# SamuelGong/FLASHE

Measured on AMD Instinct MI355X. Metric: ciphertexts/sec (enc+agg+dec), 1e7-elem vector; achieved HBM GB/s fraction, higher is better.
Workload: dtype u128

## Files before the change

flashe_amd/csrc/abi.hip:

```cpp
#include "ctx.h"
#include "blockpool.h"

#include <algorithm>
#include <cstdarg>
#include <cstdio>
#include <cstdlib>
#include <cmath>
#include <cstring>
#include <mutex>
#include <new>
#include <string>
#include <vector>

using namespace flashe;

namespace {

struct AesTables {
    uint8_t sbox[256];
    uint32_t te0[256];
    AesTables()
    {
        uint8_t alog[256], lg[256];
        uint8_t x = 1;
// ... 330 lines not shown
    ctx->env.rkw_dev = ctx->rkw_dev;
    if ((e = hipMalloc(&ctx->rkp_dev, 15 * 64 * 4)) != hipSuccess) return bail(FLASHE_ENOMEM, "hipMalloc(rkp)", e);
    ctx->env.rkp_dev = ctx->rkp_dev;
    if ((e = hipHostMalloc(reinterpret_cast<void **>(&ctx->err_flag_host), 64, hipHostMallocMapped)) != hipSuccess)
        return bail(FLASHE_ENOMEM, "hipHostMalloc(error flag)", e);
    *ctx->err_flag_host = 0;
    if ((e = hipHostGetDevicePointer(reinterpret_cast<void **>(&ctx->env.err_flag), ctx->err_flag_host, 0)) != hipSuccess)
        return bail(FLASHE_EIO, "hipHostGetDevicePointer", e);
    expand_key(key, &ctx->env.rk);
    if (upload_key_words(ctx) != FLASHE_OK) {
        g_create_error = ctx->err;
        (void)flashe_ctx_destroy(ctx);
        return FLASHE_EIO;
    }
    ctx->env.prf_backend = PRF_AUTO;
    ctx->env.hybrid_bs_permille = 300;
    if ((e = hipStreamCreateWithFlags(&ctx->env.stream2, hipStreamNonBlocking)) != hipSuccess) return bail(FLASHE_EIO, "hipStreamCreate(2)", e);
    if ((e = hipEventCreateWithFlags(&ctx->env.ev_fork, hipEventDisableTiming)) != hipSuccess) return bail(FLASHE_EIO, "hipEventCreate", e);
    if ((e = hipEventCreateWithFlags(&ctx->env.ev_join, hipEventDisableTiming)) != hipSuccess) return bail(FLASHE_EIO, "hipEventCreate", e);
    if (const char *be = getenv("FLASHE_PRF_BACKEND")) {
        if (!strcmp(be, "table")) ctx->env.prf_backend = PRF_TABLE;
#ifdef FLASHE_WITH_BITSLICE
        else if (!strcmp(be, "bitslice")) ctx->env.prf_backend = PRF_BITSLICE;
        else if (!strcmp(be, "hybrid")) ctx->env.prf_backend = PRF_HYBRID;
        else if (!strcmp(be, "bitslice16")) ctx->env.prf_backend = PRF_BITSLICE16;
#endif
    }
#ifdef FLASHE_TUNING
    if (const char *pm = getenv("FLASHE_HYBRID_BS_PERMILLE")) ctx->env.hybrid_bs_permille = atoi(pm);
#endif
    ctx->env.use_chain = 1;
    if (const char *ch = getenv("FLASHE_CHAIN")) ctx->env.use_chain = atoi(ch) != 0;
    if (const char *dm = getenv("FLASHE_CHAIN_DMASK")) ctx->chain_dmask_on = atoi(dm) != 0;
    *out = ctx;
    return FLASHE_OK;
}

int flashe_ctx_destroy(flashe_ctx *ctx)
{
    if (!ctx) return FLASHE_EINVAL;
    (void)hipSetDevice(ctx->device);
    if (ctx->env.stream) (void)hipStreamSynchronize(ctx->env.stream);
    for (flashe_ctx::Buf *b : {&ctx->summaries, &ctx->stream_tmp, &ctx->acc_tmp[0], &ctx->acc_tmp[1], &ctx->sp_ws, &ctx->bounds, &ctx->mt_ws, &ctx->codec_tab, &ctx->prep_enc.add,
                               &ctx->prep_enc.minus, &ctx->prep_dec.add, &ctx->prep_dec.minus, &ctx->chain_dmask.d})
        if (b->p) (void)hipFree(b->p);
    if (ctx->staging) { ctx->staging->destroy(); delete ctx->staging; ctx->staging = nullptr; }
    if (ctx->te0_dev) (void)hipFree(ctx->te0_dev);
    if (ctx->rkw_dev) { (void)hipMemset(ctx->rkw_dev, 0, 256); (void)hipFree(ctx->rkw_dev); }
    if (ctx->rkp_dev) { (void)hipMemset(ctx->rkp_dev, 0, 15 * 64 * 4); (void)hipFree(ctx->rkp_dev); }
    wipe(&ctx->env.rk, sizeof(ctx->env.rk));
    if (ctx->err_flag_host) (void)hipHostFree(ctx->err_flag_host);
    if (ctx->env.stream2) { (void)hipStreamSynchronize(ctx->env.stream2); (void)hipStreamDestroy(ctx->env.stream2); }
    if (ctx->env.ev_fork) (void)hipEventDestroy(ctx->env.ev_fork);
    if (ctx->env.ev_join) (void)hipEventDestroy(ctx->env.ev_join);
    for (hipEvent_t &ev : ctx->ev_copy) if (ev) (void)hipEventDestroy(ev);
    if (ctx->own_stream && ctx->env.stream) (void)hipStreamDestroy(ctx->env.stream);
    delete ctx;
    return FLASHE_OK;
}

int flashe_ctx_set_key(flashe_ctx *ctx, const uint8_t key[32])
{
    if (!ctx || !key) return FLASHE_EINVAL;
    HIP_TRY(ctx, hipSetDevice(ctx->device));
    HIP_TRY(ctx, hipStreamSynchronize(ctx->env.stream));
    wipe(&ctx->env.rk, sizeof(ctx->env.rk));
// ... 1848 lines not shown
{
    CHECK_CTX(ctx);
    if (n_layers < 0 || (n_layers && (!n || !k))) return fail(ctx, FLASHE_EINVAL, "sparsify_batch: bad arguments");
    if (n_layers == 0) return FLASHE_OK;
    if (ctx->capturing) return fail(ctx, FLASHE_EINVAL, "sparsify_batch: not inside a graph capture (the layer table is uploaded synchronously)");
    uint64_t total = 0, total_k = 0;
    for (int l = 0; l < n_layers; l++) {
        if (n[l] >= (1ull << 32)) return fail(ctx, FLASHE_EINVAL, "sparsify_batch: layer %d: n must be < 2^32", l);
        if (k[l] > n[l]) return fail(ctx, FLASHE_EINVAL, "sparsify_batch: layer %d: k (%llu) > n (%llu)", l, static_cast<unsigned long long>(k[l]),
                                     static_cast<unsigned long long>(n[l]));
        total += n[l]; total_k += k[l];
    }
    if (total == 0 || total_k == 0) return FLASHE_OK;
    if (!x_dev || !loc_dev || !vals_dev) return fail(ctx, FLASHE_EINVAL, "null vector");
    std::vector<unsigned char> desc(sparsify_batch_desc_bytes(n_layers));
    const uint64_t blocks = sparsify_batch_layout(n_layers, n, k, desc.data());
    if (blocks >= (1ull << 32)) return fail(ctx, FLASHE_EINVAL, "sparsify_batch: too many elements");
    int rc = ensure(ctx, ctx->sp_ws, sparsify_batch_workspace_bytes(n_layers, blocks));
    if (rc) return rc;
    HIP_TRY(ctx, hipMemcpyAsync(ctx->sp_ws.p, desc.data(), desc.size(), hipMemcpyHostToDevice, ctx->env.stream));
    HIP_TRY(ctx, hipStreamSynchronize(ctx->env.stream));
    HIP_TRY(ctx, launch_sparsify_batch(ctx->env, n_layers, blocks, x_dev, x_is_f64 != 0, residual_dev, loc_dev, vals_dev, ctx->sp_ws.p));
    return FLASHE_OK;
}

#ifdef FLASHE_TUNING
int flashe_tune_span_prf_cycles(flashe_ctx *ctx, unsigned long long *out8, int reset)
{
    CHECK_CTX(ctx);
    HIP_TRY(ctx, hipStreamSynchronize(ctx->env.stream));
    HIP_TRY(ctx, flashe::span_prf_cycles(out8, reset != 0));
    return FLASHE_OK;
}
int flashe_tune_reduce_decrypt_probe(flashe_ctx *ctx, int variant, uint32_t iter, uint32_t add_idx, uint32_t minus_idx, int C,
                                     const uint64_t *const *cts_dev, uint64_t n, uint64_t *out_dev)
{
    CHECK_CTX(ctx);
    if (!cts_dev || !out_dev) return fail(ctx, FLASHE_EINVAL, "null vector");
    HIP_TRY(ctx, launch_reduce_decrypt_probe(ctx->env, variant, iter, add_idx, minus_idx, C, cts_dev, n, out_dev));
    return FLASHE_OK;
}
#endif

}
```

flashe_amd/csrc/kernels.h:

```cpp
#pragma once
#include <hip/hip_runtime.h>
#include <stdint.h>

namespace flashe {

struct RoundKeys { uint32_t w[60]; };

struct CodecLayer {
    uint64_t start;
    const void *x;
    double p0, p1, p2;
    int x_is_f64, pad_;
};
struct Codec {
    const void *x;
    const double *u;
    double alpha, scale, den;
    int x_is_f64, n_layers;
    double *fout;
    double ac, two_a, uden;
    const CodecLayer *layers;
    uint64_t k0;
};

struct LaunchEnv {
    hipStream_t stream;
    int num_cus;
    const uint32_t *te0_dev;
    const uint32_t *rkw_dev;
    const uint32_t *rkp_dev;
    RoundKeys rk;
    int b;
    int prf_backend;
    hipStream_t stream2;
    hipEvent_t ev_fork, ev_join;
    int hybrid_bs_permille;
    const Codec *codec;
    uint32_t *err_flag;
    int use_chain;
    int elem32 = 0;
};

enum { PRF_AUTO = 0, PRF_TABLE = 1, PRF_BITSLICE = 2, PRF_HYBRID = 3, PRF_BITSLICE16 = 4 };

constexpr int kMaxIdx = 96;
hipError_t launch_prf(const LaunchEnv &env, uint32_t iter,
                      const uint32_t *add, int n_add, const uint32_t *minus, int n_minus,
                      uint64_t n, uint32_t n_jobs, uint64_t first, uint64_t count,
                      const uint64_t *in_dev, int in_limbs, uint64_t *out_dev);

constexpr int kMaxBatch = 32;
constexpr int kMaxUniformBatch = 128;
hipError_t launch_prf_batch(const LaunchEnv &env, uint32_t iter, bool dbl, int n_vec, const uint32_t *idx,
                            const uint64_t *const *in_dev, int in_limbs, uint64_t *const *out_dev, uint64_t n,
                            uint32_t n_jobs);
hipError_t launch_prf_batch_sum(const LaunchEnv &env, uint32_t iter, int n_vec, const uint32_t *idx, const uint64_t *const *in_dev,
                                int in_limbs, uint64_t *const *out_dev, uint64_t *sum_out_dev, uint64_t n, uint32_t n_jobs, uint64_t first,
                                uint64_t count, uint64_t *dmask_dev = nullptr);
hipError_t launch_prf_batch_range(const LaunchEnv &env, uint32_t iter, bool dbl, int n_vec, const uint32_t *idx, const uint64_t *const *in_dev,
                                  int in_limbs, uint64_t *const *out_dev, uint64_t n, uint32_t n_jobs, uint64_t first, uint64_t count);

struct PrfJob {
    uint32_t add_idx, minus_idx;
    uint64_t first, count;
    const uint64_t *in_dev;
    int in_limbs;
    uint64_t *out_dev;
    uint32_t n_in = 1;
    uint64_t in_stride = 0;
    uint64_t *sum_out_dev = nullptr;
};
hipError_t launch_prf_jobs(const LaunchEnv &env, uint32_t iter, bool dbl, int n_entries, const PrfJob *jobs, uint64_t n,
                           uint32_t n_jobs);
// ... 36 lines not shown
hipError_t launch_aggregate_packed(const LaunchEnv &env, int C, const uint64_t *const *ops,
                                   uint64_t n_limbs, uint64_t total_bits, uint64_t *out_dev,
                                   uint32_t *summaries_dev);

hipError_t launch_packed_probe(const LaunchEnv &env, uint64_t n_limbs, const uint64_t *x_dev, uint64_t *info_dev);
hipError_t launch_packed_add_carry(const LaunchEnv &env, uint64_t n_limbs, uint64_t total_bits, uint64_t cin, uint64_t *x_dev);
hipError_t launch_packed_resolve_carry(const LaunchEnv &env, uint64_t n_limbs, uint64_t total_bits, const uint64_t *infos_dev, int n_below,
                                       uint64_t *x_dev, int stride_words = 3);

hipError_t launch_pack(const LaunchEnv &env, uint64_t n, const uint64_t *in_dev, uint64_t *out_dev);
hipError_t launch_unpack(const LaunchEnv &env, uint64_t n, const uint64_t *in_dev, uint64_t *out_dev);

hipError_t launch_fill(const LaunchEnv &env, uint64_t n, uint64_t lo, uint64_t hi, uint64_t *out_dev);
hipError_t launch_scatter(const LaunchEnv &env, uint64_t total, uint64_t k, const uint32_t *loc_dev,
                          const uint64_t *vals_dev, uint64_t *out_dev, bool accumulate,
                          uint64_t sub_lo = 0, uint64_t sub_hi = 0);
constexpr int kMaxScatter = 64;
#ifndef FLASHE_SPAN_FUSED
#define FLASHE_SPAN_FUSED 1752
#endif
constexpr int kSpanReduce = 4096, kSpanFused = FLASHE_SPAN_FUSED;
uint64_t span_count(uint64_t total, int span);
inline size_t span_table_words(uint64_t total, int C) { return static_cast<size_t>(span_count(total, kSpanFused) + 1) * static_cast<size_t>(C); }
hipError_t launch_span_reduce(const LaunchEnv &env, int C, const uint32_t *const *loc_dev, const uint64_t *const *vals_dev,
                              const uint64_t *k, const uint64_t *sub, uint64_t base_lo, uint64_t base_hi, uint64_t total,
                              uint32_t *start_dev, const uint64_t *src_dev, bool negate, uint64_t *out_dev, bool bounds_ready = false);
hipError_t launch_span_bounds(const LaunchEnv &env, int C, const uint32_t *const *loc_dev, const uint64_t *k, uint64_t total, uint32_t *start_reduce_dev,
                              uint32_t *start_fused_dev);
hipError_t launch_span_prf(const LaunchEnv &env, uint32_t iter, int C, const uint32_t *idx, const uint32_t *const *loc_dev, const uint64_t *k,
                           const uint64_t *const *pt_dev, int pt_limbs, uint64_t *const *ct_dev, const uint64_t *sub, uint64_t base_lo, uint64_t base_hi,
                           uint64_t total, const uint32_t *start_dev, const uint64_t *src_dev, bool negate, uint64_t *out_dev, uint64_t first, uint64_t count);
#ifdef FLASHE_TUNING
hipError_t span_prf_cycles(unsigned long long *out8, bool reset);
#endif
hipError_t launch_sparse_edge_prf(const LaunchEnv &env, uint32_t iter, int nc, uint32_t c0, const uint32_t *const *loc_with_neighbours,
                                  const uint64_t *k_with_neighbours, uint64_t *const *va_dev, uint64_t *const *vm_dev);
hipError_t launch_shared_positions(const LaunchEnv &env, int nc, const uint32_t *const *loc_with_next, const uint64_t *k_with_next,
                                   unsigned long long *count_dev);
hipError_t launch_sel_accumulate(const LaunchEnv &env, uint64_t total, const uint8_t *sel_dev,
                                 const uint64_t *stream_dev, uint64_t *out_dev);

Codec codec_quantize_front(const void *x_dev, bool is_f64, double alpha, int bits, const double *u_dev);
void codec_unquantize_back(Codec *c, double alpha, int bits, int num_clients, double *out_dev);
CodecLayer codec_layer_front(uint64_t start, const void *x_dev, bool is_f64, double alpha, int bits);
CodecLayer codec_layer_back(uint64_t start, double alpha, int bits, int num_clients);
hipError_t launch_shift(const LaunchEnv &env, uint64_t n, void *x_dev, bool is_f64, double shift, bool wide);
int moments_grid(const LaunchEnv &env, uint64_t n);
hipError_t launch_moment(const LaunchEnv &env, uint64_t n, const void *x_dev, bool is_f64, double center, int pow, double *part_dev);
hipError_t launch_quantize(const LaunchEnv &env, uint64_t n, const void *x_dev, bool is_f64, double alpha, int bits,
                           const double *u_dev, uint64_t *q_dev);
hipError_t launch_unquantize_model(const LaunchEnv &env, uint64_t count, const uint64_t *v_dev, const Codec &cq, double *out_dev);
hipError_t launch_unquantize(const LaunchEnv &env, uint64_t n, const uint64_t *v_dev, int v_limbs, double alpha, int bits,
                             int num_clients, double *out_dev);
hipError_t launch_batch(const LaunchEnv &env, uint64_t n, const uint64_t *vals_dev, int field_bits, uint64_t *out_dev);
struct BatchLayer {
    uint64_t elem_start;
    uint64_t value_start;
    uint64_t size;
    const void *x;
    double p0, p1, p2;
    int x_is_f64, pad_;
};
hipError_t launch_quantize_batch_model(const LaunchEnv &env, const BatchLayer *layers_dev, int n_layers, int field_bits, const double *u_dev,
                                       uint64_t n_elems, uint64_t *out_dev);
hipError_t launch_unbatch_unquantize_model(const LaunchEnv &env, const BatchLayer *layers_dev, int n_layers, int field_bits, const uint64_t *in_dev,
                                           uint64_t n_values, double *out_dev);
// ... 25 lines not shown
```

flashe_amd/csrc/kernels.hip:

```cpp
#include "device_common.h"

namespace flashe {

struct IdxLists {
    uint32_t add[kMaxIdx];
    uint32_t minus[kMaxIdx];
};

struct PrfParams {
    const uint64_t *in;
    uint64_t *out;
    const uint32_t *te0;
    uint64_t n;
    uint64_t first, count;
    uint64_t blk_first, blk_count;
    uint64_t mask_lo, mask_hi;
    uint32_t iter;
    int in_limbs;
    int n_add, n_minus;
    uint32_t n_jobs;
    int b, m;
    Codec cq;
};

// ... 206 lines not shown
constexpr int kMaxLinks = 128;
struct ChainTable {
    uint64_t first[kMaxChains], count[kMaxChains];
    uint64_t wend[kMaxChains];
    uint16_t link0[kMaxChains], sbase[kMaxChains];
    uint8_t len[kMaxChains];
    uint8_t flags[kMaxChains];
    uint32_t idx[kMaxLinks + kMaxChains];
    const uint64_t *in[kMaxLinks];
    uint64_t *out[kMaxLinks];
    uint64_t *sum_out[kMaxChains];
};

__device__ __forceinline__ CtrPrefix load_prefix(const uint32_t *pre_lds, int s)
{
    const uint4 v = *reinterpret_cast<const uint4 *>(pre_lds + 4 * s);
    return CtrPrefix{{static_cast<uint32_t>(__builtin_amdgcn_readfirstlane(v.x)), static_cast<uint32_t>(__builtin_amdgcn_readfirstlane(v.y)),
                      static_cast<uint32_t>(__builtin_amdgcn_readfirstlane(v.z)), static_cast<uint32_t>(__builtin_amdgcn_readfirstlane(v.w))}};
}

__device__ __forceinline__ void loads_landed(const u128 &a, const u128 &b)
{
    asm volatile("" ::"v"(static_cast<uint64_t>(a)), "v"(static_cast<uint64_t>(a >> 64)), "v"(static_cast<uint64_t>(b)),
                 "v"(static_cast<uint64_t>(b >> 64)));
}

template <class T> __device__ __forceinline__ void swap_regs(T &a, T &b) { const T t = a; a = b; b = t; }

__device__ __forceinline__ uint64_t uniform64(uint64_t v)
{
    return static_cast<uint32_t>(__builtin_amdgcn_readfirstlane(static_cast<uint32_t>(v))) |
           (static_cast<uint64_t>(static_cast<uint32_t>(__builtin_amdgcn_readfirstlane(static_cast<uint32_t>(v >> 32)))) << 32);
}

template <int THREADS, bool SUM, bool CODEC>
__global__ __launch_bounds__(THREADS) void prf_chain_kernel(const RoundKeys rk, const ChainTable tb, int n_chains, int all_half_arg,
                                                              uint32_t iter0, uint64_t mask_lo, uint64_t mask_hi,
                                                              const uint32_t *__restrict__ te0, const Codec cq)
{
    constexpr bool DMASK = false;
    uint64_t *const dmask = nullptr;
#include "prf_chain_body.inc"
}

template <int THREADS>
__global__ __launch_bounds__(THREADS) void prf_chain_dmask_kernel(const RoundKeys rk, const ChainTable tb, int n_chains, int all_half_arg,
                                                                    uint32_t iter0, uint64_t mask_lo, uint64_t mask_hi,
                                                                    const uint32_t *__restrict__ te0, uint64_t *__restrict__ dmask)
{
    constexpr bool SUM = true, CODEC = false, DMASK = true;
    const Codec cq{};
#include "prf_chain_body.inc"
}

__device__ __forceinline__ uint64_t extract64(u128 S, int sh)
{
    return sh >= 128 ? 0ull : static_cast<uint64_t>(S >> sh);
}

constexpr int kSmallThreads = 1024;
constexpr int kTch = 8;

__global__ __launch_bounds__(kSmallThreads) void prf_small_kernel(const RoundKeys rk, const PrfParams p, const IdxLists lists)
{
    const uint32_t iter = p.iter + p.te0[kIterShiftWord];
    __shared__ uint32_t tab[kTabWords];
// ... 1508 lines not shown
static hipError_t launch_small_chains(const LaunchEnv &env, uint32_t iter, int n_chains, const PrfChain *chains, uint64_t n, uint32_t n_jobs);

#ifndef FLASHE_CHAIN_QUARTER_DEFAULT
#define FLASHE_CHAIN_QUARTER_DEFAULT 1
#endif
hipError_t launch_prf_chains(const LaunchEnv &env, uint32_t iter, int n_chains, const PrfChain *chains, uint64_t n, uint32_t n_jobs)
{
    if (env.b <= 64) return launch_small_chains(env, iter, n_chains, chains, n, n_jobs);
    struct Piece { const PrfChain *ch; int l0, l1; uint64_t tiles; };
    std::vector<Piece> pieces;
    uint64_t total_tiles = 0;
    bool summed = false;
    uint64_t *dmask = nullptr;
    for (int i = 0; i < n_chains; i++) {
        const PrfChain &c = chains[i];
        if (c.dmask_dev && (n_chains != 1 || !c.sum_out_dev || c.single)) return hipErrorInvalidValue;
        dmask = c.dmask_dev;
        if (c.count == 0 || c.n_out == 0) continue;
        if (((c.first + c.count - 1) >> 32) != (c.first >> 32)) return hipErrorNotSupported;
        if (c.sum_out_dev) { if (c.n_out > kMaxLinks) return hipErrorNotSupported; summed = true; }
        const uint64_t tiles = (c.first + c.count - (c.first & ~255ull) + 255) / 256;
        pieces.push_back(Piece{&c, 0, c.n_out, tiles});
        total_tiles += tiles;
    }
    if (pieces.empty()) return hipSuccess;
    const uint64_t waves = static_cast<uint64_t>(env.num_cus) * (kPrfThreads / 64);
    bool all_half = total_tiles < 2 * waves;
    static const bool tune = FLASHE_TUNE_ENV("FLASHE_CHAIN_TUNE") != nullptr;
    int force_parts = 0, force_grid = 0, probe = 0;
    if (tune) {
        if (const char *e = FLASHE_TUNE_ENV("FLASHE_CHAIN_HALF")) all_half = atoi(e) != 0;
        if (const char *e = FLASHE_TUNE_ENV("FLASHE_CHAIN_PARTS")) force_parts = atoi(e);
        if (const char *e = FLASHE_TUNE_ENV("FLASHE_CHAIN_GRID")) force_grid = atoi(e);
        if (const char *e = FLASHE_TUNE_ENV("FLASHE_CHAIN_PROBE")) probe = atoi(e) == 1 ? 0x100 : atoi(e) == 2 ? 0x200 : 0;
    }
    bool only_single = true;
    for (const Piece &pc : pieces) only_single &= pc.ch->single && !pc.ch->sum_out_dev;
    int single_parts = 0;
    if (only_single && all_half && !force_parts && !(tune && FLASHE_TUNE_ENV("FLASHE_CHAIN_HALF"))) {
        single_parts = static_cast<int>(std::min<uint64_t>((2 * waves + total_tiles - 1) / total_tiles, kMaxChains / pieces.size()));
        if (single_parts < 1) single_parts = 1;
        uint64_t cut_tiles = 0;
        for (const Piece &pc : pieces) cut_tiles += pc.tiles * static_cast<uint64_t>(std::min(single_parts, pc.l1));
        all_half = 2 * cut_tiles < waves;
    }
    uint64_t cuttable_tiles = 0, fixed_items = 0;
    for (const Piece &pc : pieces) {
        if (pc.l1 >= 8 && !pc.ch->sum_out_dev) cuttable_tiles += pc.tiles;
        else fixed_items += 2 * pc.tiles;
    }
    bool quarter = !env.codec && !summed && !single_parts && all_half && 4 * total_tiles <= waves && !force_parts && FLASHE_CHAIN_QUARTER_DEFAULT;
    if (tune) {
        if (const char *e = FLASHE_TUNE_ENV("FLASHE_CHAIN_QUARTER")) quarter = atoi(e) != 0 && !env.codec && !summed && !single_parts && all_half;
    }
    std::vector<Piece> cut;
    for (const Piece &pc : pieces) {
        int parts = (pc.l1 + kMaxLinks - 1) / kMaxLinks;
        if (single_parts) {
            parts = std::max(parts, std::min(single_parts, pc.l1));
        } else if (quarter && !pc.ch->sum_out_dev && pc.l1 >= 2) {
            uint64_t cut4 = 0, fixed4 = 0;
            for (const Piece &o : pieces) (o.l1 >= 2 && !o.ch->sum_out_dev ? cut4 : fixed4) += 4 * o.tiles;
            const uint64_t want = fixed4 < waves ? std::max<uint64_t>((waves - fixed4) / cut4, 1) : 1;
            parts = std::max<int>(parts, static_cast<int>(std::min<uint64_t>(want, static_cast<uint64_t>(pc.l1))));
            parts = std::min(parts, std::max(1, kMaxChains / static_cast<int>(pieces.size())));
            parts = std::max(parts, (pc.l1 + kMaxLinks - 1) / kMaxLinks);
        } else if (all_half && 2 * total_tiles < waves && !pc.ch->sum_out_dev) {
// ... 15 lines not shown
    size_t at = 0;
    while (at < cut.size()) {
        ChainTable tb{};
        int nc = 0, links = 0, streams = 0;
        uint64_t wend = 0, tiles = 0;
        while (at < cut.size() && nc < kMaxChains && links + (cut[at].l1 - cut[at].l0) <= kMaxLinks) {
            const Piece &pc = cut[at++];
            const PrfChain &c = *pc.ch;
            const int len = pc.l1 - pc.l0, ns = len + (c.single ? 0 : 1);
            tb.first[nc] = c.first; tb.count[nc] = c.count;
            tb.link0[nc] = static_cast<uint16_t>(links); tb.sbase[nc] = static_cast<uint16_t>(streams);
            tb.len[nc] = static_cast<uint8_t>(len);
            tb.flags[nc] = static_cast<uint8_t>((c.single ? 1 : 0) | (c.in_limbs == 2 ? 2 : 0));
            tb.sum_out[nc] = c.sum_out_dev;
            for (int s = 0; s < ns; s++) tb.idx[streams + s] = c.idx[pc.l0 + s];
            for (int l = 0; l < len; l++) {
                tb.in[links + l] = c.in_dev ? c.in_dev[pc.l0 + l] : nullptr;
                tb.out[links + l] = c.out_dev[pc.l0 + l];
            }
            wend += pc.tiles * static_cast<uint64_t>(ns);
            tb.wend[nc] = wend;
            tiles += pc.tiles;
            links += len; streams += ns; nc++;
        }
        const uint64_t items = quarter ? 4 * tiles : all_half ? 2 * tiles : tiles, cus = static_cast<uint64_t>(env.num_cus);
        int grid = static_cast<int>(items < cus ? items : cus);
        if (force_grid > 0) grid = force_grid;
        Codec cq{};
        if (env.codec) {
            if (cut.size() != 1 || cut[0].l1 - cut[0].l0 != 1) return hipErrorInvalidValue;
            cq = *env.codec;
        }
        if (env.codec && summed) return hipErrorInvalidValue;
        if (dmask)
            hipLaunchKernelGGL((prf_chain_dmask_kernel<kPrfThreads>), dim3(grid), dim3(kPrfThreads), 0, env.stream, env.rk, tb, nc,
                               (all_half ? 1 : 0) | (quarter ? 4 : 0) | probe, iter, lo, hi, env.te0_dev, dmask);
        else if (env.codec)
            hipLaunchKernelGGL((prf_chain_kernel<kPrfThreads, false, true>), dim3(grid), dim3(kPrfThreads), 0, env.stream, env.rk, tb, nc,
                               (all_half ? 1 : 0) | (quarter ? 4 : 0) | probe, iter, lo, hi, env.te0_dev, cq);
        else if (summed)
            hipLaunchKernelGGL((prf_chain_kernel<kPrfThreads, true, false>), dim3(grid), dim3(kPrfThreads), 0, env.stream, env.rk, tb, nc,
                               (all_half ? 1 : 0) | (quarter ? 4 : 0) | probe, iter, lo, hi, env.te0_dev, cq);
        else
            hipLaunchKernelGGL((prf_chain_kernel<kPrfThreads, false, false>), dim3(grid), dim3(kPrfThreads), 0, env.stream, env.rk, tb, nc,
                               (all_half ? 1 : 0) | (quarter ? 4 : 0) | probe, iter, lo, hi, env.te0_dev, cq);
        const hipError_t e = hipGetLastError();
        if (e != hipSuccess) return e;
    }
    return hipSuccess;
}

static SmallParams small_params_of(const LaunchEnv &env, uint32_t iter, uint64_t n, uint32_t n_jobs)
{
    SmallParams p{};
    p.n = n; p.n_jobs = n_jobs; p.iter = iter; p.b = env.b; p.m = 128 / env.b; p.te0 = env.te0_dev;
    { static const int v = FLASHE_TUNE_ENV("FLASHE_SMALL_DIRECT") ? atoi(FLASHE_TUNE_ENV("FLASHE_SMALL_DIRECT")) : 1; p.no_direct = v == 0 ? 1 : v == 2 ? 2 : 0; }
    { static const int v = FLASHE_TUNE_ENV("FLASHE_SMALL_FIXED") ? atoi(FLASHE_TUNE_ENV("FLASHE_SMALL_FIXED")) : 1; p.no_fixed_width = v == 0; }
    p.m_magic = static_cast<uint32_t>(((1ull << 32) + p.m - 1) / p.m);
    uint64_t hi;
    masks_of(env.b, &p.mask_lo, &hi);
    unsigned __int128 top = 0;
    for (int t = 0; t < p.m; t++) top |= static_cast<unsigned __int128>(1) << (env.b * t + env.b - 1);
    p.top_lo = static_cast<uint64_t>(top); p.top_hi = static_cast<uint64_t>(top >> 64);
    const uint64_t mm = p.m, d = n / n_jobs, nb1 = (d + 1 + mm - 1) / mm, nb0 = d ? (d + mm - 1) / mm : 0;
    p.nb1_magic = nb1 > 1 && nb1 < (1ull << 32) ? static_cast<uint32_t>((1ull << 32) / nb1) : 0;
    p.nb0_magic = nb0 > 1 && nb0 < (1ull << 32) ? static_cast<uint32_t>((1ull << 32) / nb0) : 0;
    return p;
}

hipError_t launch_small_reduce_decrypt(const LaunchEnv &env, uint32_t iter, uint32_t add_idx, bool has_minus, uint32_t minus_idx, uint64_t n,
                                       uint32_t n_jobs, uint64_t first, uint64_t count, int C, const uint64_t *const *ops, uint64_t *agg_out_dev,
                                       uint64_t *out_dev, int out_elem_bytes)
{
    if (env.b > 64 || env.codec || n >= (1ull << 32) || n == 0 || n_jobs == 0 || C < 1 || C > kMaxOps) return hipErrorNotSupported;
    if ((env.elem32 || out_elem_bytes == 4) && env.b > 32) return hipErrorInvalidValue;
    if (out_elem_bytes != 8 && !(out_elem_bytes == 4 && env.elem32)) return hipErrorInvalidValue;
    if (env.prf_backend != PRF_AUTO && env.prf_backend != PRF_TABLE) return hipErrorNotSupported;
    if (count == 0) return hipSuccess;
// ... 294 lines not shown
```

flashe_amd/csrc/prf_chain_body.inc:

```
    static_assert(!DMASK || (SUM && !CODEC), "the decrypt mask is written by summed chains only");
    (void)dmask;
    const uint32_t iter = iter0 + te0[kIterShiftWord];
    constexpr uint32_t WAVES = THREADS / 64;
    __shared__ uint32_t tab[kTabWords];
    __shared__ __attribute__((aligned(16))) uint32_t pre_lds[(kMaxLinks + kMaxChains) * 4];
    __shared__ uint64_t d_tlo[kMaxChains], d_cend[kMaxChains];
    int all_half = all_half_arg;
    fill_tables(tab, te0);
#ifdef FLASHE_TUNING
    if (all_half & 0x100) return;
#endif
    const LaneRegs lr = lane_regs(tab);
    const u128 mask = (static_cast<u128>(mask_hi) << 64) | mask_lo;
    {
        const int last = n_chains - 1;
        const int n_streams = tb.sbase[last] + tb.len[last] + ((tb.flags[last] & 1) ? 0 : 1);
        for (int s = threadIdx.x; s < n_streams; s += THREADS) {
            int i = 0;
            while (i < last && s >= tb.sbase[i + 1]) i++;
            const CtrPrefix c = ctr_prefix(rk, lr, iter, tb.idx[s], static_cast<uint32_t>(tb.first[i] >> 32));
            *reinterpret_cast<uint4 *>(pre_lds + 4 * s) = make_uint4(c.u[0], c.u[1], c.u[2], c.u[3]);
        }
        if (threadIdx.x < static_cast<unsigned>(n_chains)) {
            const int i = threadIdx.x;
            const uint64_t Wt = tb.wend[last], cw = i ? tb.wend[i - 1] : 0;
            const uint32_t w = tb.len[i] + ((tb.flags[i] & 1) ? 0u : 1u);
            uint64_t a, b, T;
            if (Wt <= 0xffffffffull && gridDim.x <= 0xffffu) {
                const uint32_t W32 = static_cast<uint32_t>(Wt), G = gridDim.x, g = blockIdx.x, c32 = static_cast<uint32_t>(cw);
                const uint32_t q = W32 / G, r = W32 % G;
                const uint32_t lo = q * g + r * g / G, hi = q * (g + 1) + r * (g + 1) / G;
                const uint32_t T32 = (static_cast<uint32_t>(tb.wend[i]) - c32) / w;
                const uint32_t a32 = lo > c32 ? (lo - c32 + w - 1) / w : 0, b32 = hi > c32 ? (hi - c32 + w - 1) / w : 0;
                T = T32; a = a32; b = b32;
            } else {
                const uint64_t G = gridDim.x, g = blockIdx.x;
                const uint64_t lo = Wt / G * g + (Wt % G) * g / G, hi = Wt / G * (g + 1) + (Wt % G) * (g + 1) / G;
                T = (tb.wend[i] - cw) / w;
                a = lo > cw ? (lo - cw + w - 1) / w : 0; b = hi > cw ? (hi - cw + w - 1) / w : 0;
            }
            if (a > T) a = T;
            if (b > T) b = T;
            d_tlo[i] = a; d_cend[i] = b - a;
        }
        __syncthreads();
        if (threadIdx.x == 0) {
            uint64_t acc = 0;
            for (int i = 0; i < n_chains; i++) { acc += d_cend[i]; d_cend[i] = acc; }
        }
        __syncthreads();
    }
#ifdef FLASHE_TUNING
    if (all_half & 0x200) return;
#endif
    const bool quarter = !CODEC && !SUM && (all_half & 4) != 0;
    all_half &= 1;
    const uint32_t wave = static_cast<uint32_t>(__builtin_amdgcn_readfirstlane(threadIdx.x >> 6));
    const uint32_t lane = threadIdx.x & 63u;
    const uint64_t Ng = uniform64(d_cend[n_chains - 1]);
    const uint64_t n_full = (all_half || quarter) ? 0 : Ng - Ng % WAVES;
    const uint64_t n_items = quarter ? 4 * Ng : n_full + 2 * (Ng - n_full);
    int cur = 0;
    uint64_t cbeg = 0;
    for (uint64_t q = wave; q < n_items; q += WAVES) {
        const bool whole = q < n_full;
        const uint64_t L = quarter ? (q >> 2) : whole ? q : n_full + ((q - n_full) >> 1);
        const uint32_t half = whole || quarter ? 0u : static_cast<uint32_t>((q - n_full) & 1u);
        while (L >= uniform64(d_cend[cur])) cbeg = uniform64(d_cend[cur++]);
        const uint64_t first = tb.first[cur], end = first + tb.count[cur];
        const uint64_t tj = (first & ~255ull) + 256u * (uniform64(d_tlo[cur]) + (L - cbeg)) + 128u * half +
                            (quarter ? 64u * static_cast<uint32_t>(q & 3u) : 0u);
        const int link0 = tb.link0[cur], sbase = tb.sbase[cur];
        const bool single = tb.flags[cur] & 1, in2 = tb.flags[cur] & 2;
        const int n_streams = tb.len[cur] + (single ? 0 : 1);
        if (whole) {
            const uint32_t x3 = static_cast<uint32_t>(tj) ^ rk.w[3];
            const uint32_t jl = static_cast<uint32_t>(tj) + lane;
            uint32_t vA0 = T3(jl ^ rk.w[3], SEL_B0), vA1 = T3((jl + 64u) ^ rk.w[3], SEL_B0);
            uint32_t vB0 = T3((jl + 128u) ^ rk.w[3], SEL_B0), vB1 = T3((jl + 192u) ^ rk.w[3], SEL_B0);
            u128 pA0 = 0, pA1 = 0, pB0 = 0, pB1 = 0;
            u128 qA0 = 0, qA1 = 0, qB0 = 0, qB1 = 0;
            u128 dA0 = 0, dA1 = 0, dB0 = 0, dB1 = 0;
            uint64_t *const sum_out = SUM ? tb.sum_out[cur] : nullptr;
            for (int c = 0; c < n_streams; c++) {
                const CtrPrefix pre = load_prefix(pre_lds, sbase + c);
                const CtrUniform U = ctr_uniform(rk, te0, pre, x3);
                const int link = single ? c : c - 1;
                const uint64_t *in = link >= 0 ? tb.in[link0 + link] : nullptr;
                uint64_t *out = link >= 0 ? tb.out[link0 + link] : nullptr;
                const bool last_stream = c == n_streams - 1;
#pragma unroll 1
                for (int p = 0; p < 2; p++) {
                    const uint64_t jb = tj + 128u * p;
                    if (jb < end && jb + 128u > first) {
                        const uint64_t j0 = jb + lane, j1 = j0 + 64u, k0 = j0 - first, k1 = j1 - first;
                        const bool a0 = j0 >= first && j0 < end, a1 = j1 >= first && j1 < end;
                        u128 x0 = 0, x1 = 0;
                        if (CODEC && cq.x != nullptr && link >= 0) {
                            if (a0) x0 = codec_quantize(cq, k0);
                            if (a1) x1 = codec_quantize(cq, k1);
                        } else if (in != nullptr && in2) {
                            if (a0) x0 = ld128(in + 2 * k0);
                            if (a1) x1 = ld128(in + 2 * k1);
                        } else if (in != nullptr) {
// ... 17 lines not shown
                        if constexpr (SUM) {
                            if (link >= 0) {
                                if (p == 0) { qA0 += r0; qA1 += r1; } else { qB0 += r0; qB1 += r1; }
                            }
                            if (last_stream && sum_out != nullptr) {
                                if (p == 0) {
                                    if (a0) st128_nt(sum_out + 2 * k0, qA0 & mask);
                                    if (a1) st128_nt(sum_out + 2 * k1, qA1 & mask);
                                } else {
                                    if (a0) st128_nt(sum_out + 2 * k0, qB0 & mask);
                                    if (a1) st128_nt(sum_out + 2 * k1, qB1 & mask);
                                }
                            }
                        }
                        if constexpr (DMASK) {
                            if (c == 0) {
                                if (p == 0) { dA0 = c0; dA1 = c1; } else { dB0 = c0; dB1 = c1; }
                            }
                            if (last_stream) {
                                if (p == 0) {
                                    if (a0) st128_nt(dmask + 2 * k0, (c0 - dA0) & mask);
                                    if (a1) st128_nt(dmask + 2 * k1, (c1 - dA1) & mask);
                                } else {
                                    if (a0) st128_nt(dmask + 2 * k0, (c0 - dB0) & mask);
                                    if (a1) st128_nt(dmask + 2 * k1, (c1 - dB1) & mask);
                                }
                            }
                        }
                        pA0 = c0; pA1 = c1;
                    }
                    swap_regs(pA0, pB0); swap_regs(pA1, pB1); swap_regs(vA0, vB0); swap_regs(vA1, vB1);
                }
            }
        } else if (quarter) {
            if (!CODEC && !SUM && tj < end && tj + 64u > first) {
                const uint64_t j0 = tj + lane, k0 = j0 - first;
                const bool a0 = j0 >= first && j0 < end;
                const uint32_t x3 = static_cast<uint32_t>(tj) ^ rk.w[3];
                const uint32_t v0 = T3(static_cast<uint32_t>(j0) ^ rk.w[3], SEL_B0);
                u128 pv = 0;
                for (int c = 0; c < n_streams; c += 2) {
                    const bool has1 = c + 1 < n_streams;
                    const CtrPrefix pre0 = load_prefix(pre_lds, sbase + c), pre1 = load_prefix(pre_lds, sbase + (has1 ? c + 1 : c));
                    const CtrUniform U0 = ctr_uniform(rk, te0, pre0, x3), U1 = ctr_uniform(rk, te0, pre1, x3);
                    const int l0 = single ? c : c - 1;
                    const uint64_t *in0 = l0 >= 0 ? tb.in[link0 + l0] : nullptr, *in1 = has1 ? tb.in[link0 + l0 + 1] : nullptr;
                    u128 x0 = 0, x1 = 0;
                    if (in0 != nullptr && a0) x0 = in2 ? ld128(in0 + 2 * k0) : static_cast<u128>(in0[k0]);
                    if (in1 != nullptr && a0) x1 = in2 ? ld128(in1 + 2 * k0) : static_cast<u128>(in1[k0]);
                    uint32_t s[2][4];
                    ctr_round2(lr, pre0.u[0], v0, U0, s[0]);
                    ctr_round2(lr, pre1.u[0], v0, U1, s[1]);
                    aes256_rounds<2, 3>(rk, lr, s, FLASHE_SWP_PRIO_HALF != 0);
                    loads_landed(x0, x1);
                    const u128 c0 = words_to_u128(s[0]), c1 = words_to_u128(s[1]);
                    if (l0 >= 0) {
                        const u128 r0 = (x0 + (single ? c0 : pv - c0)) & mask;
                        if (a0 && tb.out[link0 + l0] != nullptr) st128(tb.out[link0 + l0] + 2 * k0, r0);
                    }
                    if (has1) {
                        const u128 r1 = (x1 + (single ? c1 : c0 - c1)) & mask;
                        if (a0 && tb.out[link0 + l0 + 1] != nullptr) st128(tb.out[link0 + l0 + 1] + 2 * k0, r1);
                    }
                    pv = has1 ? c1 : c0;
                }
            }
        } else if (tj < end && tj + 128u > first) {
            const uint64_t j0 = tj + lane, j1 = j0 + 64u, k0 = j0 - first, k1 = j1 - first;
            const bool a0 = j0 >= first && j0 < end, a1 = j1 >= first && j1 < end;
            const CtrVar xv0 = ctr_var(rk, lr, static_cast<uint32_t>(j0)), xv1 = ctr_var(rk, lr, static_cast<uint32_t>(j1));
#if FLASHE_HALF_U
            const uint32_t x3h = static_cast<uint32_t>(tj) ^ rk.w[3];
#endif
            u128 p0 = 0, p1 = 0, q0 = 0, q1 = 0;
            uint64_t *const sum_out = SUM ? tb.sum_out[cur] : nullptr;
            u128 d0 = 0, d1 = 0;
            for (int c = 0; c < n_streams; c++) {
                const CtrPrefix pre = load_prefix(pre_lds, sbase + c);
                const int link = single ? c : c - 1;
                const uint64_t *in = link >= 0 ? tb.in[link0 + link] : nullptr;
                uint64_t *out = link >= 0 ? tb.out[link0 + link] : nullptr;
                u128 x0 = 0, x1 = 0;
                if (CODEC && cq.x != nullptr && link >= 0) {
                    if (a0) x0 = codec_quantize(cq, k0);
                    if (a1) x1 = codec_quantize(cq, k1);
                } else if (in != nullptr && in2) {
                    if (a0) x0 = ld128(in + 2 * k0);
                    if (a1) x1 = ld128(in + 2 * k1);
                } else if (in != nullptr) {
                    if (a0) x0 = static_cast<u128>(in[k0]);
                    if (a1) x1 = static_cast<u128>(in[k1]);
                }
                uint32_t s[2][4];
#if FLASHE_HALF_U
                {
                    const CtrUniform U = ctr_uniform(rk, te0, pre, x3h);
                    ctr_round2(lr, pre.u[0], xv0.v[0], U, s[0]);
// ... 3 lines not shown
#else
                ctr_round1(pre, xv0, s[0]);
                ctr_round1(pre, xv1, s[1]);
                aes256_rounds<2, 2>(rk, lr, s, FLASHE_SWP_PRIO_HALF != 0);
#endif
                loads_landed(x0, x1);
                const u128 c0 = words_to_u128(s[0]), c1 = words_to_u128(s[1]);
                const u128 r0 = x0 + (single ? c0 : p0 - c0), r1 = x1 + (single ? c1 : p1 - c1);
                if (CODEC && cq.fout != nullptr) {
                    if (a0 && link >= 0) cq.fout[k0] = codec_unquantize(cq, k0, r0 & mask);
                    if (a1 && link >= 0) cq.fout[k1] = codec_unquantize(cq, k1, r1 & mask);
                } else {
                    if (a0 && out != nullptr) st128(out + 2 * k0, r0 & mask);
                    if (a1 && out != nullptr) st128(out + 2 * k1, r1 & mask);
                }
                if constexpr (SUM) {
                    if (link >= 0) { q0 += r0; q1 += r1; }
                    if (c == n_streams - 1 && sum_out != nullptr) {
                        if (a0) st128_nt(sum_out + 2 * k0, q0 & mask);
                        if (a1) st128_nt(sum_out + 2 * k1, q1 & mask);
                    }
                }
                if constexpr (DMASK) {
                    if (c == 0) { d0 = c0; d1 = c1; }
                    if (c == n_streams - 1) {
                        if (a0) st128_nt(dmask + 2 * k0, (c0 - d0) & mask);
                        if (a1) st128_nt(dmask + 2 * k1, (c1 - d1) & mask);
                    }
                }
                p0 = c0; p1 = c1;
            }
        }
    }
```

Before: 68.20 billion.

## Add dynamic work-claiming and quarter-split tail items to chain PRF kernel

Replaces the static wave-strided loop in the chain PRF kernel with an LDS-ticket dynamic claim, enabled by default. The tail is also split into half and quarter items, and quarter items now support the SUM and DMASK variants. The aim is to reduce load imbalance and tail idleness across waves within a block. In exchange it adds per-item atomic contention in LDS and readfirstlane overhead, and it adds a tuning-only timing probe.

New measurement: 69.74 billion, median of 6. Within noise of the previous version (+2.3%).

```diff
diff --git a/flashe_amd/csrc/abi.hip b/flashe_amd/csrc/abi.hip
--- a/flashe_amd/csrc/abi.hip
+++ b/flashe_amd/csrc/abi.hip
@@ -386,6 +386,7 @@
     ctx->env.use_chain = 1;
     if (const char *ch = getenv("FLASHE_CHAIN")) ctx->env.use_chain = atoi(ch) != 0;
     if (const char *dm = getenv("FLASHE_CHAIN_DMASK")) ctx->chain_dmask_on = atoi(dm) != 0;
+    if (const char *dy = getenv("FLASHE_CHAIN_DYN")) ctx->env.chain_dyn = atoi(dy) != 0;
     *out = ctx;
     return FLASHE_OK;
 }
@@ -2300,6 +2301,14 @@
     HIP_TRY(ctx, flashe::span_prf_cycles(out8, reset != 0));
     return FLASHE_OK;
 }
+int flashe_tune_chain_wave_ends(flashe_ctx *ctx, unsigned long long *out, int waves, int reset)
+{
+    CHECK_CTX(ctx);
+    if (!out) return fail(ctx, FLASHE_EINVAL, "null output");
+    HIP_TRY(ctx, hipStreamSynchronize(ctx->env.stream));
+    HIP_TRY(ctx, flashe::chain_probe_read(out, waves, reset != 0));
+    return FLASHE_OK;
+}
 int flashe_tune_reduce_decrypt_probe(flashe_ctx *ctx, int variant, uint32_t iter, uint32_t add_idx, uint32_t minus_idx, int C,
                                      const uint64_t *const *cts_dev, uint64_t n, uint64_t *out_dev)
 {
diff --git a/flashe_amd/csrc/kernels.h b/flashe_amd/csrc/kernels.h
--- a/flashe_amd/csrc/kernels.h
+++ b/flashe_amd/csrc/kernels.h
@@ -39,6 +39,7 @@
     uint32_t *err_flag;
     int use_chain;
     int elem32 = 0;
+    int chain_dyn = 1;
 };
 
 enum { PRF_AUTO = 0, PRF_TABLE = 1, PRF_BITSLICE = 2, PRF_HYBRID = 3, PRF_BITSLICE16 = 4 };
@@ -141,6 +142,7 @@
                            uint64_t total, const uint32_t *start_dev, const uint64_t *src_dev, bool negate, uint64_t *out_dev, uint64_t first, uint64_t count);
 #ifdef FLASHE_TUNING
 hipError_t span_prf_cycles(unsigned long long *out8, bool reset);
+hipError_t chain_probe_read(unsigned long long *out, int waves, bool reset);
 #endif
 hipError_t launch_sparse_edge_prf(const LaunchEnv &env, uint32_t iter, int nc, uint32_t c0, const uint32_t *const *loc_with_neighbours,
                                   const uint64_t *k_with_neighbours, uint64_t *const *va_dev, uint64_t *const *vm_dev);
diff --git a/flashe_amd/csrc/kernels.hip b/flashe_amd/csrc/kernels.hip
--- a/flashe_amd/csrc/kernels.hip
+++ b/flashe_amd/csrc/kernels.hip
@@ -262,6 +262,44 @@
     return static_cast<uint32_t>(__builtin_amdgcn_readfirstlane(static_cast<uint32_t>(v))) |
            (static_cast<uint64_t>(static_cast<uint32_t>(__builtin_amdgcn_readfirstlane(static_cast<uint32_t>(v >> 32)))) << 32);
 }
+
+__device__ __forceinline__ uint32_t claim_item(uint32_t *ticket)
+{
+    uint32_t t = 0;
+    if ((threadIdx.x & 63u) == 0) t = __hip_atomic_fetch_add(ticket, 1u, __ATOMIC_RELAXED, __HIP_MEMORY_SCOPE_WORKGROUP);
+    return static_cast<uint32_t>(__builtin_amdgcn_readfirstlane(t));
+}
+
+#ifdef FLASHE_TUNING
+constexpr int kChainProbeWaves = 8192;
+__device__ unsigned long long g_chain_probe[kChainProbeWaves * 4];
+__device__ __forceinline__ void chain_probe_record(uint64_t t0, uint32_t items)
+{
+    const uint64_t t1 = __builtin_amdgcn_s_memrealtime();
+    uint32_t xcc, hw;
+    asm volatile("s_getreg_b32 %0, hwreg(HW_REG_XCC_ID)" : "=s"(xcc));
+    asm volatile("s_getreg_b32 %0, hwreg(HW_REG_HW_ID)" : "=s"(hw));
+    const uint32_t w = blockIdx.x * (blockDim.x >> 6) + (threadIdx.x >> 6);
+    if ((threadIdx.x & 63u) == 0 && w < static_cast<uint32_t>(kChainProbeWaves)) {
+        unsigned long long *const r = g_chain_probe + 4 * w;
+        r[0] = t0; r[1] = t1;
+        r[2] = (static_cast<unsigned long long>(xcc) << 32) | hw;
+        r[3] = (static_cast<unsigned long long>(items) << 32) | blockIdx.x;
+    }
+}
+
+hipError_t chain_probe_read(unsigned long long *out, int waves, bool reset)
+{
+    if (waves < 0 || waves > kChainProbeWaves) return hipErrorInvalidValue;
+    hipError_t e = hipMemcpyFromSymbol(out, HIP_SYMBOL(g_chain_probe), static_cast<size_t>(waves) * 4 * sizeof(unsigned long long));
+    if (e == hipSuccess && reset) {
+        void *p = nullptr;
+        e = hipGetSymbolAddress(&p, HIP_SYMBOL(g_chain_probe));
+        if (e == hipSuccess) e = hipMemset(p, 0, sizeof g_chain_probe);
+    }
+    return e;
+}
+#endif
 
 template <int THREADS, bool SUM, bool CODEC>
 __global__ __launch_bounds__(THREADS) void prf_chain_kernel(const RoundKeys rk, const ChainTable tb, int n_chains, int all_half_arg,
@@ -1836,7 +1874,7 @@
         if (const char *e = FLASHE_TUNE_ENV("FLASHE_CHAIN_HALF")) all_half = atoi(e) != 0;
         if (const char *e = FLASHE_TUNE_ENV("FLASHE_CHAIN_PARTS")) force_parts = atoi(e);
         if (const char *e = FLASHE_TUNE_ENV("FLASHE_CHAIN_GRID")) force_grid = atoi(e);
-        if (const char *e = FLASHE_TUNE_ENV("FLASHE_CHAIN_PROBE")) probe = atoi(e) == 1 ? 0x100 : atoi(e) == 2 ? 0x200 : 0;
+        if (const char *e = FLASHE_TUNE_ENV("FLASHE_CHAIN_PROBE")) probe = atoi(e) == 1 ? 0x100 : atoi(e) == 2 ? 0x200 : atoi(e) == 3 ? 0x400 : 0;
     }
     bool only_single = true;
     for (const Piece &pc : pieces) only_single &= pc.ch->single && !pc.ch->sum_out_dev;
@@ -1918,18 +1956,20 @@
             cq = *env.codec;
         }
         if (env.codec && summed) return hipErrorInvalidValue;
+        const int flags = (all_half ? 1 : 0) | (quarter ? 4 : 0) | (env.chain_dyn ? 8 : 0) | probe;
+        const unsigned lds = env.chain_dyn ? sizeof(uint32_t) : 0u;
         if (dmask)
-            hipLaunchKernelGGL((prf_chain_dmask_kernel<kPrfThreads>), dim3(grid), dim3(kPrfThreads), 0, env.stream, env.rk, tb, nc,
-                               (all_half ? 1 : 0) | (quarter ? 4 : 0) | probe, iter, lo, hi, env.te0_dev, dmask);
+            hipLaunchKernelGGL((prf_chain_dmask_kernel<kPrfThreads>), dim3(grid), dim3(kPrfThreads), lds, env.stream, env.rk, tb, nc,
+                               flags, iter, lo, hi, env.te0_dev, dmask);
         else if (env.codec)
-            hipLaunchKernelGGL((prf_chain_kernel<kPrfThreads, false, true>), dim3(grid), dim3(kPrfThreads), 0, env.stream, env.rk, tb, nc,
-                               (all_half ? 1 : 0) | (quarter ? 4 : 0) | probe, iter, lo, hi, env.te0_dev, cq);
+            hipLaunchKernelGGL((prf_chain_kernel<kPrfThreads, false, true>), dim3(grid), dim3(kPrfThreads), lds, env.stream, env.rk, tb, nc,
+                               flags, iter, lo, hi, env.te0_dev, cq);
         else if (summed)
-            hipLaunchKernelGGL((prf_chain_kernel<kPrfThreads, true, false>), dim3(grid), dim3(kPrfThreads), 0, env.stream, env.rk, tb, nc,
-                               (all_half ? 1 : 0) | (quarter ? 4 : 0) | probe, iter, lo, hi, env.te0_dev, cq);
+            hipLaunchKernelGGL((prf_chain_kernel<kPrfThreads, true, false>), dim3(grid), dim3(kPrfThreads), lds, env.stream, env.rk, tb, nc,
+                               flags, iter, lo, hi, env.te0_dev, cq);
         else
-            hipLaunchKernelGGL((prf_chain_kernel<kPrfThreads, false, false>), dim3(grid), dim3(kPrfThreads), 0, env.stream, env.rk, tb, nc,
-                               (all_half ? 1 : 0) | (quarter ? 4 : 0) | probe, iter, lo, hi, env.te0_dev, cq);
+            hipLaunchKernelGGL((prf_chain_kernel<kPrfThreads, false, false>), dim3(grid), dim3(kPrfThreads), lds, env.stream, env.rk, tb, nc,
+                               flags, iter, lo, hi, env.te0_dev, cq);
         const hipError_t e = hipGetLastError();
         if (e != hipSuccess) return e;
     }
diff --git a/flashe_amd/csrc/prf_chain_body.inc b/flashe_amd/csrc/prf_chain_body.inc
--- a/flashe_amd/csrc/prf_chain_body.inc
+++ b/flashe_amd/csrc/prf_chain_body.inc
@@ -5,7 +5,11 @@
     __shared__ uint32_t tab[kTabWords];
     __shared__ __attribute__((aligned(16))) uint32_t pre_lds[(kMaxLinks + kMaxChains) * 4];
     __shared__ uint64_t d_tlo[kMaxChains], d_cend[kMaxChains];
+    extern __shared__ uint32_t chain_ticket[];
     int all_half = all_half_arg;
+#ifdef FLASHE_TUNING
+    const uint64_t probe_t0 = __builtin_amdgcn_s_memrealtime();
+#endif
     fill_tables(tab, te0);
 #ifdef FLASHE_TUNING
     if (all_half & 0x100) return;
@@ -43,6 +47,7 @@
             if (b > T) b = T;
             d_tlo[i] = a; d_cend[i] = b - a;
         }
+        if ((all_half & 8) && threadIdx.x == 0) chain_ticket[0] = WAVES;
         __syncthreads();
         if (threadIdx.x == 0) {
             uint64_t acc = 0;
@@ -53,23 +58,38 @@
 #ifdef FLASHE_TUNING
     if (all_half & 0x200) return;
 #endif
-    const bool quarter = !CODEC && !SUM && (all_half & 4) != 0;
+    const bool quarter = !CODEC && (all_half & 4) != 0;
+    const bool dyn_arg = (all_half & 8) != 0;
     all_half &= 1;
     const uint32_t wave = static_cast<uint32_t>(__builtin_amdgcn_readfirstlane(threadIdx.x >> 6));
     const uint32_t lane = threadIdx.x & 63u;
-    const uint64_t Ng = uniform64(d_cend[n_chains - 1]);
-    const uint64_t n_full = (all_half || quarter) ? 0 : Ng - Ng % WAVES;
-    const uint64_t n_items = quarter ? 4 * Ng : n_full + 2 * (Ng - n_full);
+    const uint32_t Ng = static_cast<uint32_t>(uniform64(d_cend[n_chains - 1]));
+    uint32_t n_full, n_qt;
+    if (quarter) { n_full = 0; n_qt = Ng; }
+    else if (all_half) { n_full = 0; n_qt = 0; }
+    else if (dyn_arg) {
+        const uint32_t tail = Ng < Ng % WAVES + WAVES ? Ng : Ng % WAVES + WAVES;
+        n_full = Ng - tail;
+        n_qt = CODEC ? 0 : (tail < WAVES / 2 ? tail : WAVES / 2);
+    } else { n_full = Ng - Ng % WAVES; n_qt = 0; }
+    const uint32_t n_half = Ng - n_full - n_qt, q0 = n_full + 2 * n_half;
+    const uint32_t n_items = q0 + 4 * n_qt;
+#ifdef FLASHE_TUNING
+    uint32_t probe_items = 0;
+#endif
     int cur = 0;
     uint64_t cbeg = 0;
-    for (uint64_t q = wave; q < n_items; q += WAVES) {
-        const bool whole = q < n_full;
-        const uint64_t L = quarter ? (q >> 2) : whole ? q : n_full + ((q - n_full) >> 1);
-        const uint32_t half = whole || quarter ? 0u : static_cast<uint32_t>((q - n_full) & 1u);
+    for (uint32_t q = wave; q < n_items; q = dyn_arg ? claim_item(chain_ticket) : q + WAVES) {
+#ifdef FLASHE_TUNING
+        probe_items++;
+#endif
+        const bool whole = q < n_full, qitem = !CODEC && q >= q0;
+        const uint32_t L = whole ? q : qitem ? n_full + n_half + ((q - q0) >> 2) : n_full + ((q - n_full) >> 1);
+        const uint32_t half = whole || qitem ? 0u : static_cast<uint32_t>((q - n_full) & 1u);
         while (L >= uniform64(d_cend[cur])) cbeg = uniform64(d_cend[cur++]);
         const uint64_t first = tb.first[cur], end = first + tb.count[cur];
         const uint64_t tj = (first & ~255ull) + 256u * (uniform64(d_tlo[cur]) + (L - cbeg)) + 128u * half +
-                            (quarter ? 64u * static_cast<uint32_t>(q & 3u) : 0u);
+                            (qitem ? 64u * static_cast<uint32_t>((q - q0) & 3u) : 0u);
         const int link0 = tb.link0[cur], sbase = tb.sbase[cur];
         const bool single = tb.flags[cur] & 1, in2 = tb.flags[cur] & 2;
         const int n_streams = tb.len[cur] + (single ? 0 : 1);
@@ -153,13 +173,14 @@
                     swap_regs(pA0, pB0); swap_regs(pA1, pB1); swap_regs(vA0, vB0); swap_regs(vA1, vB1);
                 }
             }
-        } else if (quarter) {
-            if (!CODEC && !SUM && tj < end && tj + 64u > first) {
+        } else if (qitem) {
+            if (tj < end && tj + 64u > first) {
                 const uint64_t j0 = tj + lane, k0 = j0 - first;
                 const bool a0 = j0 >= first && j0 < end;
                 const uint32_t x3 = static_cast<uint32_t>(tj) ^ rk.w[3];
                 const uint32_t v0 = T3(static_cast<uint32_t>(j0) ^ rk.w[3], SEL_B0);
                 u128 pv = 0;
+                u128 qs = 0, d0 = 0;
                 for (int c = 0; c < n_streams; c += 2) {
                     const bool has1 = c + 1 < n_streams;
                     const CtrPrefix pre0 = load_prefix(pre_lds, sbase + c), pre1 = load_prefix(pre_lds, sbase + (has1 ? c + 1 : c));
@@ -178,12 +199,23 @@
                     if (l0 >= 0) {
                         const u128 r0 = (x0 + (single ? c0 : pv - c0)) & mask;
                         if (a0 && tb.out[link0 + l0] != nullptr) st128(tb.out[link0 + l0] + 2 * k0, r0);
+                        if constexpr (SUM) qs += r0;
                     }
                     if (has1) {
                         const u128 r1 = (x1 + (single ? c1 : c0 - c1)) & mask;
                         if (a0 && tb.out[link0 + l0 + 1] != nullptr) st128(tb.out[link0 + l0 + 1] + 2 * k0, r1);
+                        if constexpr (SUM) qs += r1;
+                    }
+                    if constexpr (DMASK) {
+                        if (c == 0) d0 = c0;
                     }
                     pv = has1 ? c1 : c0;
+                }
+                if constexpr (SUM) {
+                    if (a0 && tb.sum_out[cur] != nullptr) st128_nt(tb.sum_out[cur] + 2 * k0, qs & mask);
+                }
+                if constexpr (DMASK) {
+                    if (a0) st128_nt(dmask + 2 * k0, (pv - d0) & mask);
                 }
             }
         } else if (tj < end && tj + 128u > first) {
@@ -253,3 +285,6 @@
             }
         }
     }
+#ifdef FLASHE_TUNING
+    if (all_half_arg & 0x400) chain_probe_record(probe_t0, probe_items);
+#endif
```
